# powei-lin/camera-intrinsic-calibration-rs

Measured on AMD Instinct MI355X. Metric: corner residual+Jacobian evals/sec; LM iters/sec to converge (EUCM, TUM-VI cam0), higher is better.
Workload: dtype f64

## Files before the change

### camera_intrinsic_calibration_rs_amd/csrc/ccal_api.hip

```cpp
#include <algorithm>
#include <cmath>
#include <cstdio>
#include <cstring>
#include <memory>
#include <new>

#include "ccal_internal.hpp"
#include "ccal_normal.hpp"

using namespace ccal;

#define HIP_TRY(ctx, expr)                                                                         \
    do {                                                                                           \
        hipError_t e_ = (expr);                                                                    \
        if (e_ != hipSuccess) {                                                                    \
            (ctx)->err = std::string(#expr) + ": " + hipGetErrorString(e_);                        \
            return CCAL_ERR_HIP;                                                                   \
        }                                                                                          \
    } while (0)

static void stream_synced(ccal_problem* p) {
    if (!p->nws) return;
    p->nws->tail_pending = false;
    if (p->nws->fws) p->nws->fws->tail_pending = false;
}

static int fail(ccal_ctx* ctx, int code, const char* msg) {
    if (ctx) ctx->err = msg;
    return code;
}

template <class T>
static int upload(ccal_ctx* ctx, T** dst, const T* src, size_t n) {
    HIP_TRY(ctx, hipMalloc((void**)dst, (n + 1) * sizeof(T)));
    if (n) HIP_TRY(ctx, hipMemcpyAsync(*dst, src, n * sizeof(T), hipMemcpyHostToDevice, ctx->stream));
    HIP_TRY(ctx, hipMemsetAsync(*dst + n, 0, sizeof(T), ctx->stream));
    return CCAL_OK;
}

// ... 164 lines not shown
        p->h_obs_off.assign(1, 0);
    }
    p->h_joff.resize(d->n_obs + 1);
    std::vector<uint8_t> seen((size_t)d->n_cams * (size_t)std::max(d->n_slots, 1), 0);
    int64_t j = 0;
    for (int o = 0; o < d->n_obs; ++o) {
        const int cam = p->h_obs_cam[o], slot = p->h_obs_slot[o];
        const int64_t n = p->h_obs_off[o + 1] - p->h_obs_off[o];
        if (cam < 0 || cam >= d->n_cams || slot < 0 || slot >= d->n_slots || n < 0 || p->h_obs_off[0] != 0)
            return fail(ctx, CCAL_ERR_INVALID_ARG, "bad observation frame table");
        uint8_t& sn = seen[(size_t)cam * d->n_slots + slot];
        if (sn) return fail(ctx, CCAL_ERR_INVALID_ARG, "two observation frames for the same (camera, slot)");
        sn = 1;
        p->h_joff[o] = j; j += n * 2 * p->cams[cam].D;
        p->cams[cam].obs.push_back(o);
    }
    p->h_joff[d->n_obs] = j; p->j_len = j;
    p->slot_ident = d->n_slots == d->n_obs;
    for (int o = 0; o < d->n_obs && p->slot_ident; ++o) p->slot_ident = p->h_obs_slot[o] == o;
    p->n_corners = p->h_obs_off[d->n_obs];
    if (p->n_corners >= ((int64_t)1 << 30)) return fail(ctx, CCAL_ERR_INVALID_ARG, "more than 2^30 - 1 corners in one problem: shard the frames (ccal_multi_problem_create)");
    const size_t nc = (size_t)p->n_corners;
    if (nc && (!d->p3d_x || !d->p3d_y || !d->p3d_z || !d->p2d_u || !d->p2d_v)) return fail(ctx, CCAL_ERR_INVALID_ARG, "null corner arrays");
    {
        uint32_t any = 0;
        for (size_t i = 0; i < nc; ++i) { uint32_t b; std::memcpy(&b, d->p3d_z + i, sizeof b); any |= b & 0x7fffffffu; }
        p->has_nonplanar = any != 0;
    }
    const size_t ni = (size_t)d->n_cams * CCAL_PMAX, np6 = (size_t)std::max(d->n_slots, 1) * 6, ne = (size_t)d->n_cams * 6;
    auto up256 = [](size_t b) { return (b + 255) & ~(size_t)255; };
    size_t total = 5 * up256((nc + 1) * sizeof(float)) + 2 * up256((p->h_obs_off.size() + 1) * sizeof(int64_t)) +
                   2 * up256((p->h_obs_cam.size() + 1) * sizeof(int32_t)) + 2 * (up256(ni * 8) + up256(np6 * 8) + up256(ne * 8));
    for (int c = 0; c < d->n_cams; ++c) total += up256((p->cams[c].obs.size() + 1) * sizeof(int32_t));
    std::vector<int32_t> bin_tab;
    if (d->n_cams == 1 && d->n_obs > 0) {
        std::vector<int32_t> order;
        const int m0 = p->cams[0].model;
        p->gram_bins = gram2_bin_plan(p->h_obs_off.data(), d->n_obs, m0 == kUCM || m0 == kEUCM, &order);
        if (p->gram_bins.n_bins > 0) {
            bin_tab.assign((size_t)d->n_obs * 4 + 4, 0);
            for (int i = 0; i < d->n_obs; ++i) {
                const int o = order[(size_t)i];
                bin_tab[4 * (size_t)i] = o; bin_tab[4 * (size_t)i + 1] = (int32_t)p->h_obs_off[o];
                bin_tab[4 * (size_t)i + 2] = (int32_t)(p->h_obs_off[o + 1] - p->h_obs_off[o]); bin_tab[4 * (size_t)i + 3] = p->h_obs_slot[o];
            }
            total += up256((bin_tab.size() + 1) * sizeof(int32_t));
        }
    }
    HIP_TRY(ctx, ctx_dev_alloc(ctx, (void**)&p->d_block, total));
    char* h_pack = nullptr;
    struct PackGuard { ccal_ctx* c; char*& p; ~PackGuard() { if (p) { (void)hipStreamSynchronize(c->stream); ccal::ctx_release(c, p, true); } } } pack_guard{ ctx, h_pack };
    if (total <= ((size_t)8 << 20)) HIP_TRY(ctx, ctx_host_alloc(ctx, (void**)&h_pack, total));
    if (!h_pack) HIP_TRY(ctx, hipMemsetAsync(p->d_block, 0, total, ctx->stream));
    {
        char* q = p->d_block;
        auto put = [&](auto** dst, const auto* src, size_t n) -> hipError_t {
            using T = std::remove_pointer_t<std::remove_pointer_t<decltype(dst)>>;
            *dst = reinterpret_cast<T*>(q);
            const size_t room = up256((n + 1) * sizeof(T));
            if (h_pack) {
                char* h = h_pack + (q - p->d_block);
                const size_t nb = (n && src) ? n * sizeof(T) : 0;
                if (nb) std::memcpy(h, src, nb);
                std::memset(h + nb, 0, room - nb);
                q += room;
                return hipSuccess;
            }
            q += room;
            return (n && src) ? hipMemcpyAsync(*dst, src, n * sizeof(T), hipMemcpyHostToDevice, ctx->stream) : hipSuccess;
        };
        HIP_TRY(ctx, put(&p->d_x, d->p3d_x, nc)); HIP_TRY(ctx, put(&p->d_y, d->p3d_y, nc)); HIP_TRY(ctx, put(&p->d_z, d->p3d_z, nc));
        HIP_TRY(ctx, put(&p->d_u, d->p2d_u, nc)); HIP_TRY(ctx, put(&p->d_v, d->p2d_v, nc));
        HIP_TRY(ctx, put(&p->d_obs_off, (const int64_t*)p->h_obs_off.data(), p->h_obs_off.size()));
        HIP_TRY(ctx, put(&p->d_joff, (const int64_t*)p->h_joff.data(), p->h_joff.size()));
        HIP_TRY(ctx, put(&p->d_obs_cam, (const int32_t*)p->h_obs_cam.data(), p->h_obs_cam.size()));
        HIP_TRY(ctx, put(&p->d_obs_slot, (const int32_t*)p->h_obs_slot.data(), p->h_obs_slot.size()));
        for (int c = 0; c < d->n_cams; ++c) HIP_TRY(ctx, put(&p->cams[c].d_obs, (const int32_t*)p->cams[c].obs.data(), p->cams[c].obs.size()));
        if (!bin_tab.empty()) HIP_TRY(ctx, put(&p->d_bin_tab, (const int32_t*)bin_tab.data(), bin_tab.size()));
        double** bufs[6] = { &p->d_intr, &p->d_poses, &p->d_extr, &p->d_intr_c, &p->d_poses_c, &p->d_extr_c };
        const size_t sz[6] = { ni, np6, ne, ni, np6, ne };
        const size_t packed = (size_t)(q - p->d_block);
        for (int i = 0; i < 6; ++i) { *bufs[i] = reinterpret_cast<double*>(q); q += up256(sz[i] * 8); }
        if ((size_t)(q - p->d_block) > total) return fail(ctx, CCAL_ERR_HIP, "problem block layout");
        if (h_pack) {
            HIP_TRY(ctx, hipMemcpyAsync(p->d_block, h_pack, packed, hipMemcpyHostToDevice, ctx->stream));
            HIP_TRY(ctx, hipMemsetAsync(p->d_block + packed, 0, total - packed, ctx->stream));
        }
    }
    p->lo.assign(ni, 0.0); p->hi.assign(ni, 0.0); p->has_bound.assign(ni, 0); p->fixed.assign(ni, 0);
    if (hipStreamSynchronize(ctx->stream) != hipSuccess) return fail(ctx, CCAL_ERR_HIP, "upload failed");
    p->counted = true;
    ctx->n_problems += 1;
    *out = hold.release();
    return CCAL_OK;
    CCAL_API_CATCH(ctx)
}

void ccal_problem_destroy(ccal_problem* p) {
    if (!p) return;
    if (p->nws && p->ctx && (p->nws->tail_pending || (p->nws->fws && p->nws->fws->tail_pending))) {
        (void)hipSetDevice(p->ctx->device);
        (void)hipDeviceSynchronize();
        p->nws->tail_pending = false;
        if (p->nws->fws) p->nws->fws->tail_pending = false;
    }
    ccal_ctx* ctx = p->ctx;
    if (ctx && (p->d_block || p->nws)) {
        (void)hipSetDevice(ctx->device);
        if (ctx->own_stream && ctx->stream) (void)hipStreamSynchronize(ctx->stream); else (void)hipDeviceSynchronize();
        (void)hipGetLastError();
    }
    void* ptrs[] = { p->d_block, p->d_r, p->d_J, p->d_err, p->d_scratch };
    for (void* q : ptrs) if (q) ctx_release(ctx, q, false);
    normal_ws_destroy(p);
    const bool counted = p->counted;
    delete p;
    if (ctx && counted && --ctx->n_problems == 0 && ctx->destroy_requested) ctx_free(ctx);
}

int64_t ccal_num_corners(const ccal_problem* p) { return p ? p->n_corners : -1; }
// ... 37 lines not shown
            const int at = cl.model == kOCV5 ? 4 + cv.ocv5_order[i - 4] : i;
            ccal_set_bounds(p, c, at - shift, cv.dist_lo[cl.model][i - 4], cv.dist_hi[cl.model][i - 4]);
        }
    }
    return CCAL_OK;
}
int ccal_disable_distortions(ccal_problem* p, int n_disabled, double* intr_io) {
    if (!p || n_disabled < 0) return CCAL_ERR_INVALID_ARG;
    const int shift = p->one_focal ? 1 : 0;
    for (int c = 0; c < p->n_cams; ++c) {
        for (int i = 0; i < n_disabled; ++i) {
            const int eff = p->cams[c].P - 1 - shift - i;
            if (eff < 0) return CCAL_ERR_INVALID_ARG;
            ccal_fix_param(p, c, eff);
            if (intr_io) intr_io[c * CCAL_PMAX + eff + shift] = 0.0;
        }
    }
    return CCAL_OK;
}
int ccal_set_allreduce(ccal_problem* p, ccal_allreduce_fn fn, void* user) {
    if (!p) return CCAL_ERR_INVALID_ARG;
    if (p->allreduce != fn || p->allreduce_user != user) { const int rc = drain_pending_groups(p); if (rc != CCAL_OK) return rc; }
    p->allreduce = fn; p->allreduce_user = user;
    return CCAL_OK;
}

int ccal_upload_params(ccal_problem* p, const double* intr, const double* poses, const double* extr) {
    if (!p) return CCAL_ERR_INVALID_ARG;
    ccal_ctx* ctx = p->ctx;
    HIP_TRY(ctx, hipSetDevice(ctx->device));
    if (intr) HIP_TRY(ctx, hipMemcpyAsync(p->d_intr, intr, sizeof(double) * p->n_cams * CCAL_PMAX, hipMemcpyHostToDevice, ctx->stream));
    if (poses && p->n_slots) HIP_TRY(ctx, hipMemcpyAsync(p->d_poses, poses, sizeof(double) * p->n_slots * 6, hipMemcpyHostToDevice, ctx->stream));
    if (extr) HIP_TRY(ctx, hipMemcpyAsync(p->d_extr, extr, sizeof(double) * p->n_cams * 6, hipMemcpyHostToDevice, ctx->stream));
    HIP_TRY(ctx, hipStreamSynchronize(ctx->stream));
    stream_synced(p);
    return CCAL_OK;
}
int ccal_download_params(ccal_problem* p, double* intr, double* poses, double* extr) {
    if (!p) return CCAL_ERR_INVALID_ARG;
    ccal_ctx* ctx = p->ctx;
    HIP_TRY(ctx, hipSetDevice(ctx->device));
    if (intr) HIP_TRY(ctx, hipMemcpyAsync(intr, p->d_intr, sizeof(double) * p->n_cams * CCAL_PMAX, hipMemcpyDeviceToHost, ctx->stream));
    if (poses && p->n_slots) HIP_TRY(ctx, hipMemcpyAsync(poses, p->d_poses, sizeof(double) * p->n_slots * 6, hipMemcpyDeviceToHost, ctx->stream));
    if (extr) HIP_TRY(ctx, hipMemcpyAsync(extr, p->d_extr, sizeof(double) * p->n_cams * 6, hipMemcpyDeviceToHost, ctx->stream));
    HIP_TRY(ctx, hipStreamSynchronize(ctx->stream));
    stream_synced(p);
    if (intr && p->one_focal) for (int c = 0; c < p->n_cams; ++c) intr[c * CCAL_PMAX + 1] = intr[c * CCAL_PMAX];
    return CCAL_OK;
}

static KArgs make_args(const ccal_problem* p, int cam) {
    KArgs a = {};
    a.x = p->d_x; a.y = p->d_y; a.z = p->d_z; a.u = p->d_u; a.v = p->d_v;
    a.obs_off = p->d_obs_off; a.obs_slot = p->d_obs_slot; a.joff = p->d_joff;
    a.list = p->cams[cam].d_obs; a.n_list = (int32_t)p->cams[cam].obs.size(); a.cam = cam;
    a.intr = p->d_intr; a.poses = p->d_poses; a.extr = p->d_extr;
    a.huber_delta = p->huber_delta; a.rt = model_rt(p->ctx);
    return a;
}

int ccal_eval_dev(ccal_problem* p, int apply_loss, double* r_dev, double* J_dev) {
    if (!p || !r_dev || !J_dev) return CCAL_ERR_INVALID_ARG;
    ccal_ctx* ctx = p->ctx;
    HIP_TRY(ctx, hipSetDevice(ctx->device));
    for (int c = 0; c < p->n_cams; ++c) {
        KArgs a = make_args(p, c);
        a.apply_loss = apply_loss; a.r_out = r_dev; a.J_out = J_dev;
        HIP_TRY(ctx, launch_eval(p, c, a, ctx->stream));
    }
    return CCAL_OK;
}

int ccal_eval(ccal_problem* p, const double* intr, const double* poses, const double* extr,
              int apply_loss, double* r_out, double* J_out) {
    if (!p || !intr || (!poses && p->n_slots) || (!extr && p->n_cams > 1) || !r_out || !J_out) return CCAL_ERR_INVALID_ARG;
    ccal_ctx* ctx = p->ctx;
    int rc = ccal_upload_params(p, intr, poses, extr);
    if (rc != CCAL_OK) return rc;
    if (!p->d_r) {
        HIP_TRY(ctx, ctx_dev_alloc(ctx, (void**)&p->d_r, sizeof(double) * std::max<int64_t>(2 * p->n_corners, 2)));
        HIP_TRY(ctx, test_poison_f64(ctx, p->d_r, sizeof(double) * std::max<int64_t>(2 * p->n_corners, 2), false, ctx->stream));
    }
    if (!p->d_J) {
        HIP_TRY(ctx, ctx_dev_alloc(ctx, (void**)&p->d_J, sizeof(double) * std::max<int64_t>(p->j_len, 2)));
        HIP_TRY(ctx, test_poison_f64(ctx, p->d_J, sizeof(double) * std::max<int64_t>(p->j_len, 2), false, ctx->stream));
    }
    rc = ccal_eval_dev(p, apply_loss, p->d_r, p->d_J);
    if (rc != CCAL_OK) return rc;
    if (p->n_corners) {
        HIP_TRY(ctx, hipMemcpyAsync(r_out, p->d_r, sizeof(double) * 2 * p->n_corners, hipMemcpyDeviceToHost, ctx->stream));
        HIP_TRY(ctx, hipMemcpyAsync(J_out, p->d_J, sizeof(double) * p->j_len, hipMemcpyDeviceToHost, ctx->stream));
    }
    HIP_TRY(ctx, hipStreamSynchronize(ctx->stream));
    return CCAL_OK;
}

}
// ... 76 lines not shown
```

### camera_intrinsic_calibration_rs_amd/csrc/ccal_internal.hpp

```cpp
#pragma once
#include <hip/hip_runtime.h>

#include <atomic>
#include <cstdint>
#include <exception>
#include <functional>
#include <mutex>
#include <new>
#include <string>
#include <vector>

#include "../../include/ccal.h"
#include "ccal_models.hpp"

namespace ccal {

constexpr int WAVES_PER_BLOCK = 4;
constexpr int PF_STRIDE = 64;

struct KArgs {
    const float* x; const float* y; const float* z; const float* u; const float* v;
    const int64_t* obs_off;
    const int32_t* obs_slot;
    const int64_t* joff;
    const int32_t* list;
    int32_t n_list;
    int32_t cam;
    const double* intr;
    const double* poses;
    const double* extr;
    double huber_delta;
    ModelRt rt;
    int32_t apply_loss;
    double* r_out;
    double* J_out;
    double* err_out;
};

struct NormalWs;

struct CamLayout {
    int model = 0, P = 0, Peff = 0, D = 0;
    int col_theta = 0, col_extr = -1;
    double width = 0, height = 0;
    std::vector<int32_t> obs;
    int32_t* d_obs = nullptr;
};

}

struct ccal_ctx {
    int device = 0;
    hipStream_t stream = nullptr;
    bool own_stream = false;
    std::string err;
    ccal_model_conventions conv;
    int n_problems = 0;
    bool destroy_requested = false;
    struct ccal_ctx_worker* worker = nullptr;
    char* d_batch_tab = nullptr; char* h_batch_tab = nullptr; size_t batch_tab_bytes = 0;
    std::vector<std::pair<void*, size_t>> pinned;
    struct Block { void* p; size_t bytes; };
    std::vector<Block> cache_dev, cache_host;
    std::vector<hipStream_t> cache_streams;
    std::vector<std::pair<void*, std::pair<size_t, int>>> live;
};
namespace ccal {
constexpr size_t kCacheDevMaxBytes = (size_t)1 << 30, kCacheHostMaxBytes = (size_t)64 << 20;
constexpr size_t kCacheMaxBlocks = 12;
// ... 81 lines not shown
}

namespace ccal {
constexpr int kGramMaxBins = 5;
struct GramBins {
    int32_t n_bins = 0;
    int32_t lpf[kGramMaxBins] = {}, first[kGramMaxBins] = {}, count[kGramMaxBins] = {}, wg0[kGramMaxBins + 1] = {};
    int32_t fold = 0;
};
GramBins gram2_bin_plan(const int64_t* obs_off, int n_obs, bool two_per_simd, std::vector<int32_t>* order, bool rig_list = false);

}

struct ccal_problem {
    ccal_ctx* ctx = nullptr;
    int n_cams = 0, n_slots = 0, n_obs = 0, K = 0;
    bool one_focal = false;
    double huber_delta = 1.0;
    int64_t n_corners = 0, j_len = 0;
    std::vector<ccal::CamLayout> cams;
    std::vector<int64_t> h_obs_off, h_joff;
    std::vector<int32_t> h_obs_cam, h_obs_slot;
    bool slot_ident = false;
    bool has_nonplanar = false;
    ccal::GramBins gram_bins;
    int32_t* d_bin_tab = nullptr;
    char* d_scratch = nullptr; size_t scratch_bytes = 0;
    char* d_block = nullptr;
    float *d_x = nullptr, *d_y = nullptr, *d_z = nullptr, *d_u = nullptr, *d_v = nullptr;
    int64_t *d_obs_off = nullptr, *d_joff = nullptr;
    int32_t *d_obs_cam = nullptr, *d_obs_slot = nullptr;
    double *d_intr = nullptr, *d_poses = nullptr, *d_extr = nullptr;
    double *d_intr_c = nullptr, *d_poses_c = nullptr, *d_extr_c = nullptr;
    std::vector<double> lo, hi;
    std::vector<uint8_t> has_bound, fixed;
    ccal::NormalWs* nws = nullptr;
    double *d_r = nullptr, *d_J = nullptr, *d_err = nullptr;
    ccal_allreduce_fn allreduce = nullptr;
    void* allreduce_user = nullptr;
    void* rccl_comm = nullptr;
    void* peer = nullptr;
    bool counted = false;
    bool sharded() const { return allreduce != nullptr || rccl_comm != nullptr || peer != nullptr; }
};

#define CCAL_API_TRY try {
#define CCAL_API_CATCH(ctx_expr)                                                                   \
    }                                                                                              \
    catch (const std::bad_alloc&) { ccal::note_error((ctx_expr), "out of host memory"); return CCAL_ERR_NO_MEMORY; }  \
    catch (const std::exception& e_) { ccal::note_error((ctx_expr), e_.what()); return CCAL_ERR_HIP; }                \
    catch (...) { ccal::note_error((ctx_expr), "unknown C++ exception"); return CCAL_ERR_HIP; }

namespace ccal {
inline void note_error(ccal_ctx* ctx, const char* msg) noexcept {
    if (!ctx) return;
    try { ctx->err = msg; } catch (...) { }
}
inline void note_error(const ccal_ctx*, const char*) noexcept {}
hipError_t launch_eval(const ccal_problem* p, int cam, const KArgs& a, hipStream_t s);
hipError_t launch_reproj_err(const ccal_problem* p, int cam, const KArgs& a, hipStream_t s);
int rccl_allreduce_sum(ccal_ctx* ctx, void* comm, double* buf, size_t count, hipStream_t st);
int drain_pending_groups(ccal_problem* p);
inline size_t problem_scratch_hint(const ccal_problem* p) {
    return (size_t)std::max<int64_t>(p->n_corners, 1) * 32 + (size_t)(std::max(p->n_obs, 1) + 1) * 64 + (size_t)384 * 1024;
}
hipError_t validation_stats_device(ccal_problem* p, int cam, const double* d_err, double* avg_99, double* median, hipStream_t s);
hipError_t camera_errors_device(ccal_problem* p, int cam, const double* d_err, double** d_out, int64_t* n_out, hipStream_t s);
size_t order_stats_block_bytes(int64_t n, hipStream_t s);
hipError_t order_stats_block(char* block , size_t block_bytes, int64_t n, double* avg_99, double* median, hipStream_t s);
int reprojection_errors_dev(ccal_problem* p, const double* intr, const double* poses, const double* extr);
hipError_t launch_pose_init(const ccal_problem* p, int cam, const double* d_intr, double* d_poses_obs, int32_t* d_valid,
                            int min_points, hipStream_t s);
hipError_t launch_pose_init_division(const ccal_problem* p, int cam, double lambda, double* d_poses_obs, int32_t* d_valid,
                                     int min_points, hipStream_t s);
hipError_t launch_pose_pnp(const ccal_problem* p, int cam, const double* d_intr, double* d_poses_obs, int32_t* d_valid,
                           int min_points, hipStream_t s);
hipError_t launch_pose_pnp_division(const ccal_problem* p, int cam, double lambda, double* d_poses_obs, int32_t* d_valid,
                                    int min_points, hipStream_t s);
hipError_t launch_pnp_batch(int n_prob, const int64_t* d_off, const double* d_xyz, const double* d_xn, int min_points,
                            double* d_poses, int32_t* d_n_used, double* d_cost, hipStream_t s);
struct DynLdsGuard { std::atomic<size_t> enabled[16] = {}; };
inline std::mutex& dyn_lds_mutex() { static std::mutex m; return m; }
inline hipError_t ensure_dyn_lds(const void* fn, size_t lds, DynLdsGuard& g) {
    if (lds <= 48 * 1024) return hipSuccess;
    int dev = 0;
    hipError_t e = hipGetDevice(&dev);
    if (e != hipSuccess) return e;
    std::atomic<size_t>& have = g.enabled[dev & 15];
    if (lds <= have.load(std::memory_order_acquire)) return hipSuccess;
    std::lock_guard<std::mutex> lk(dyn_lds_mutex());
    if (lds <= have.load(std::memory_order_relaxed)) return hipSuccess;
    e = hipFuncSetAttribute(fn, hipFuncAttributeMaxDynamicSharedMemorySize, (int)lds);
    if (e == hipSuccess) have.store(lds, std::memory_order_release);
// ... 25 lines not shown
```

### camera_intrinsic_calibration_rs_amd/csrc/ccal_kernels_eval.hip

```cpp
#include "ccal_device.hpp"
#include "ccal_internal.hpp"

#include <algorithm>
#include <type_traits>

namespace ccal {

__device__ __forceinline__ void wave_lds_sync() {
    __builtin_amdgcn_fence(__ATOMIC_RELEASE, "wavefront");
    __builtin_amdgcn_wave_barrier();
    __builtin_amdgcn_fence(__ATOMIC_ACQUIRE, "wavefront");
}

#ifndef CCAL_EVAL_WPB
#define CCAL_EVAL_WPB 2
#endif
#ifndef CCAL_EVAL_NT
#define CCAL_EVAL_NT 1
#endif
#ifndef CCAL_EVAL_NTR
#define CCAL_EVAL_NTR 0
#endif
#ifndef CCAL_EVAL_PREFETCH
#define CCAL_EVAL_PREFETCH -1
#endif
#ifndef CCAL_EVAL_PERSIST
#define CCAL_EVAL_PERSIST 0
#endif

constexpr int eval_tile_stride(int D) { return 2 * D + ((D & 1) ? 4 : 2); }
template <bool OTHER> constexpr int fc_doubles() { return OTHER ? FC_SIZE : FC_N0P; }

template <int MODEL, bool OF, bool OTHER, bool PF, bool AL>
__global__ __launch_bounds__(64 * CCAL_EVAL_WPB) void k_eval(const KArgs a) {
    constexpr int D = block_dim(MODEL, OF, OTHER);
    constexpr int TW = 2 * D;
    constexpr int TS = eval_tile_stride(D);
    constexpr int FCN = fc_doubles<OTHER>();
    constexpr int WS = FCN + 64 * TS;
    extern __shared__ double smem[];
    const int wave = threadIdx.x >> 6, lane = threadIdx.x & 63;
    double* fc = smem + wave * WS;
    double* tile = fc + FCN;
    const int wstride = CCAL_EVAL_PERSIST > 0 ? (int)gridDim.x * CCAL_EVAL_WPB : a.n_list;
    for (int widx = blockIdx.x * CCAL_EVAL_WPB + wave; widx < a.n_list; widx += wstride) {
    const int o = __builtin_amdgcn_readfirstlane(a.list[widx]);
    const int slot = __builtin_amdgcn_readfirstlane(a.obs_slot[o]);
    const int64_t start = a.obs_off[o];
    const int n = (int)(a.obs_off[o + 1] - start);
    const double* th_g = a.intr + a.cam * CCAL_PMAX;
    double th[th_len<MODEL>()];
    load_theta<MODEL, OF>(th_g, a.rt, th);

    float pX = 0.f, pY = 0.f, pZ = 0.f, pU = 0.f, pV = 0.f;
    if constexpr (PF) {
        if (n > 0) {
            const int64_t g0 = start + (lane < n ? lane : 0);
            pX = a.x[g0]; pY = a.y[g0]; pZ = a.z[g0]; pU = a.u[g0]; pV = a.v[g0];
        }
    }
    {
        double pose[6], ex[6];
#pragma unroll
        for (int i = 0; i < 6; ++i) pose[i] = a.poses[(int64_t)slot * 6 + i];
        if constexpr (OTHER) {
#pragma unroll
            for (int i = 0; i < 6; ++i) ex[i] = a.extr[a.cam * 6 + i];
        }
        double fcr[OTHER ? FC_SIZE : FC_N0];
        frame_setup<OTHER>(pose, ex, fcr);
        if (lane == 0) {
#pragma unroll
            for (int i = 0; i < (OTHER ? FC_SIZE : FC_N0); ++i) fc[i] = fcr[i];
        }
    }
    wave_lds_sync();

    const int64_t jbase = a.joff[o];
    auto pass = [&](auto full_tag, const int base) {
        constexpr bool FULL = decltype(full_tag)::value;
        const int c = base + lane;
        const bool valid = FULL || c < n;
        const int64_t g = start + (valid ? c : 0);
        double X, Y, Z, uo, vo;
        if constexpr (PF) {
            X = pX; Y = pY; Z = pZ; uo = pU; vo = pV;
            if (base + 64 < n) {
                const int cn = base + 64 + lane;
                const int64_t gn = start + (cn < n ? cn : 0);
                pX = a.x[gn]; pY = a.y[gn]; pZ = a.z[gn]; pU = a.u[gn]; pV = a.v[gn];
            }
        } else {
            X = a.x[g]; Y = a.y[g]; Z = a.z[g]; uo = a.u[g]; vo = a.v[g];
        }
        double ru, rv, J[TW];
        double* Ju = J;
        double* Jv = J + D;
#if defined(CCAL_EVAL_DIAG) && CCAL_EVAL_DIAG == 2
        ru = X + uo; rv = Y + vo;
#pragma unroll
        for (int i = 0; i < D; ++i) { Ju[i] = X * (double)(i + 1) + fc[0]; Jv[i] = Z * (double)(i + 1) + vo; }
#else
        corner_block<MODEL, OF, OTHER>(th, fc, X, Y, Z, uo, vo, ru, rv, Ju, Jv);
#endif
        if constexpr (AL) {
            const double sw = huber_sqrt_weight(ru * ru + rv * rv, a.huber_delta);
            ru *= sw; rv *= sw;
#pragma unroll
            for (int i = 0; i < D; ++i) { Ju[i] *= sw; Jv[i] *= sw; }
// ... 14 lines not shown
                    const int at = D0 + ocv5_pos(a.rt.ocv5_perm, i);
                    row[at] = J[D0 + i]; row[D + at] = J[D + D0 + i];
                }
            }
        }
        wave_lds_sync();
        double* dst = a.J_out + jbase + (int64_t)base * TW;
        auto put = [&](const int e) {
            const int cr = e / TW;
            const int k = e - cr * TW;
            const double2 val = *reinterpret_cast<const double2*>(tile + cr * TS + k);
#if defined(CCAL_EVAL_DIAG) && CCAL_EVAL_DIAG == 1
            if (e != lane * 2 || val.x != 12345.678) return;
#endif
#if CCAL_EVAL_NT
            __builtin_nontemporal_store(val.x, dst + e);
            __builtin_nontemporal_store(val.y, dst + e + 1);
#else
            *reinterpret_cast<double2*>(dst + e) = val;
#endif
        };
        if constexpr (FULL) {
#pragma unroll
            for (int it = 0; it < TW / 2; ++it) put(lane * 2 + 128 * it);
        } else {
            const int tot = (n - base) * TW;
            for (int e = lane * 2; e < tot; e += 128) put(e);
        }
        wave_lds_sync();
    };
    const int n_full = n & ~63;
    for (int base = 0; base < n_full; base += 64) pass(std::true_type{}, base);
    if (n_full < n) pass(std::false_type{}, n_full);
    }
}

template <int MODEL, bool OF, bool OTHER>
__global__ __launch_bounds__(256) void k_reproj_err(const KArgs a) {
    constexpr int FCN = fc_doubles<OTHER>();
    __shared__ double smem[WAVES_PER_BLOCK * FCN];
    const int wave = threadIdx.x >> 6, lane = threadIdx.x & 63;
    const int widx = blockIdx.x * WAVES_PER_BLOCK + wave;
    if (widx >= a.n_list) return;
    double* fc = smem + wave * FCN;
    const int o = __builtin_amdgcn_readfirstlane(a.list[widx]);
    const int slot = __builtin_amdgcn_readfirstlane(a.obs_slot[o]);
    const int64_t start = a.obs_off[o];
    const int n = (int)(a.obs_off[o + 1] - start);
    const double* th_g = a.intr + a.cam * CCAL_PMAX;
    double th[th_len<MODEL>()];
    load_theta<MODEL, OF>(th_g, a.rt, th);
    {
        double pose[6], ex[6];
#pragma unroll
        for (int i = 0; i < 6; ++i) pose[i] = a.poses[(int64_t)slot * 6 + i];
        if constexpr (OTHER) {
#pragma unroll
            for (int i = 0; i < 6; ++i) ex[i] = a.extr[a.cam * 6 + i];
        }
        double fcr[OTHER ? FC_SIZE : FC_N0];
        frame_setup<OTHER>(pose, ex, fcr);
        if (lane == 0) {
#pragma unroll
            for (int i = 0; i < 12; ++i) fc[i] = fcr[i];
        }
    }
    wave_lds_sync();
    for (int c = lane; c < n; c += 64) {
        const int64_t g = start + c;
        double px, py, pz, u, v;
        transform_point(fc, a.x[g], a.y[g], a.z[g], px, py, pz);
        project_uv<MODEL>(th, px, py, pz, u, v);
        const double du = u - (double)a.u[g], dv = v - (double)a.v[g];
        a.err_out[g] = sqrt(du * du + dv * dv);
    }
}

template <int MODEL, bool OF, bool OTHER, bool PF, bool AL>
static hipError_t launch_eval_pf(const KArgs& a, hipStream_t s) {
    constexpr int D = block_dim(MODEL, OF, OTHER);
    constexpr int WS = fc_doubles<OTHER>() + 64 * eval_tile_stride(D);
    const size_t lds = sizeof(double) * WS * CCAL_EVAL_WPB;
    int blocks = (a.n_list + CCAL_EVAL_WPB - 1) / CCAL_EVAL_WPB;
    if (blocks == 0) return hipSuccess;
    if (CCAL_EVAL_PERSIST > 0) blocks = std::min(blocks, 256 * CCAL_EVAL_PERSIST);
    static DynLdsGuard lds_guard;
    if (hipError_t e = ensure_dyn_lds(reinterpret_cast<const void*>(&k_eval<MODEL, OF, OTHER, PF, AL>), lds, lds_guard); e != hipSuccess) return e;
    hipLaunchKernelGGL((k_eval<MODEL, OF, OTHER, PF, AL>), dim3(blocks), dim3(64 * CCAL_EVAL_WPB), lds, s, a);
    return hipGetLastError();
}
#ifndef CCAL_EVAL_PF_MIN_D
#define CCAL_EVAL_PF_MIN_D 99
#endif
template <int MODEL, bool OF, bool OTHER> constexpr bool eval_prefetch_always() { return block_dim(MODEL, OF, OTHER) >= CCAL_EVAL_PF_MIN_D; }
template <int MODEL, bool OF, bool OTHER>
static hipError_t launch_eval_t(const KArgs& a, bool big_inputs, hipStream_t s) {
    const bool pf = CCAL_EVAL_PREFETCH < 0 ? (big_inputs || eval_prefetch_always<MODEL, OF, OTHER>()) : CCAL_EVAL_PREFETCH != 0;
    if (a.apply_loss) return pf ? launch_eval_pf<MODEL, OF, OTHER, true, true>(a, s) : launch_eval_pf<MODEL, OF, OTHER, false, true>(a, s);
    return pf ? launch_eval_pf<MODEL, OF, OTHER, true, false>(a, s) : launch_eval_pf<MODEL, OF, OTHER, false, false>(a, s);
}
template <int MODEL, bool OF, bool OTHER>
static hipError_t launch_err_t(const KArgs& a, hipStream_t s) {
    const int blocks = (a.n_list + WAVES_PER_BLOCK - 1) / WAVES_PER_BLOCK;
    if (blocks == 0) return hipSuccess;
    hipLaunchKernelGGL((k_reproj_err<MODEL, OF, OTHER>), dim3(blocks), dim3(256), 0, s, a);
    return hipGetLastError();
}

#define CCAL_DISPATCH(FN, model, of, other, ...)                                                     \
    do {                                                                                             \
        const int key_ = (model) * 4 + ((of) ? 2 : 0) + ((other) ? 1 : 0);                           \
        switch (key_) {                                                                              \
            case 0: return FN<kUCM, false, false>(__VA_ARGS__);   case 1: return FN<kUCM, false, true>(__VA_ARGS__);   \
            case 2: return FN<kUCM, true, false>(__VA_ARGS__);    case 3: return FN<kUCM, true, true>(__VA_ARGS__);    \
            case 4: return FN<kEUCM, false, false>(__VA_ARGS__);  case 5: return FN<kEUCM, false, true>(__VA_ARGS__);  \
            case 6: return FN<kEUCM, true, false>(__VA_ARGS__);   case 7: return FN<kEUCM, true, true>(__VA_ARGS__);   \
            case 8: return FN<kKB4, false, false>(__VA_ARGS__);   case 9: return FN<kKB4, false, true>(__VA_ARGS__);   \
            case 10: return FN<kKB4, true, false>(__VA_ARGS__);   case 11: return FN<kKB4, true, true>(__VA_ARGS__);   \
            case 12: return FN<kOCV5, false, false>(__VA_ARGS__); case 13: return FN<kOCV5, false, true>(__VA_ARGS__); \
            case 14: return FN<kOCV5, true, false>(__VA_ARGS__);  case 15: return FN<kOCV5, true, true>(__VA_ARGS__);  \
            default: return hipErrorInvalidValue;                                                    \
        }                                                                                            \
    } while (0)

hipError_t launch_eval(const ccal_problem* p, int cam, const KArgs& a, hipStream_t s) {
    const bool big_inputs = p->n_corners * 20 > (int64_t)120 << 20;
    CCAL_DISPATCH(launch_eval_t, p->cams[cam].model, p->one_focal, cam > 0, a, big_inputs, s);
}
hipError_t launch_reproj_err(const ccal_problem* p, int cam, const KArgs& a, hipStream_t s) {
    CCAL_DISPATCH(launch_err_t, p->cams[cam].model, p->one_focal, cam > 0, a, s);
}

}
```

### camera_intrinsic_calibration_rs_amd/csrc/ccal_solver.hip

```cpp
#include <algorithm>
#include <chrono>
#include <cmath>
#include <cstdio>
#include <cstring>

#include <cstdlib>
#include <atomic>
#include <condition_variable>
#include <functional>
#include <memory>
#include <mutex>
#include <thread>

#include "ccal_fused.hpp"
#include "ccal_devopt.hpp"

using namespace ccal;

#define HIP_TRYN(ctx, expr)                                                                        \
    do {                                                                                           \
        hipError_t e_ = (expr);                                                                    \
        if (e_ != hipSuccess) {                                                                    \
            (ctx)->err = std::string(#expr) + ": " + hipGetErrorString(e_);                        \
            return -CCAL_ERR_HIP;                                                                  \
        }                                                                                          \
    } while (0)

#define HIP_TRY(ctx, expr)                                                                         \
    do {                                                                                           \
        hipError_t e_ = (expr);                                                                    \
        if (e_ != hipSuccess) {                                                                    \
            (ctx)->err = std::string(#expr) + ": " + hipGetErrorString(e_);                        \
            return CCAL_ERR_HIP;                                                                   \
        }                                                                                          \
    } while (0)

namespace ccal {

hipError_t test_poison_f64(ccal_ctx* ctx, void* p, size_t bytes, bool host, hipStream_t s) {
#ifdef CCAL_TEST_HOOKS
    const char* e = std::getenv("CCAL_TEST_POISON_ALLOC");
    if (!e || e[0] != '1' || !p || !bytes) return hipSuccess;
    if (host) { std::memset(p, 0xFF, bytes); return hipSuccess; }
    return hipMemsetAsync(p, 0xFF, bytes, s ? s : ctx->stream);
#else
    (void)ctx; (void)p; (void)bytes; (void)host; (void)s;
    return hipSuccess;
#endif
}

void normal_ws_destroy(ccal_problem* p) {
    NormalWs* w = p->nws;
    if (!w) return;
    if (w->tail_pending || (w->fws && w->fws->tail_pending)) {
        (void)hipSetDevice(p->ctx->device);
        (void)hipDeviceSynchronize();
    }
    void* ptrs[] = { w->G[0], w->G[1], w->cost_o[0], w->cost_o[1], w->d_goff, w->d_slot_off, w->d_slot_obs, w->d_obs_cam,
                     w->d_caminfo, w->partial, w->red, w->pf, w->dc, w->mc_slot, w->scal, w->flags, w->cols, w->d_slot_desc, w->d_slot_rec, w->d_all_obs, w->d_obs_owner };
    ccal_ctx* ctx = p->ctx;
    for (void* q : ptrs) if (q) ctx_release(ctx, q, false);
    for (int32_t* q : w->d_gen_sorted) if (q) ctx_release(ctx, q, false);
    if (w->h_pinned) (void)hipHostFree(w->h_pinned);
    if (w->d_gstate) ctx_release(ctx, w->d_gstate, false);
    if (w->side) { (void)hipStreamSynchronize(w->side); ctx_stream_put(ctx, w->side); }
    if (w->h_gstatus) ctx_release(ctx, w->h_gstatus, true);
    if (w->h_gstate) (void)hipHostFree(w->h_gstate);
    if (FusedWs* f = w->fws) {
        if (f->side) { (void)hipStreamSynchronize(f->side); ctx_stream_put(ctx, f->side); }
        if (f->d_block) ctx_release(ctx, f->d_block, false);
        if (f->h_block) ctx_release(ctx, f->h_block, true);
        if (f->fcbuf) (void)hipFree(f->fcbuf);
        delete f;
    }
    delete w;
    p->nws = nullptr;
}

int drain_pending_groups(ccal_problem* p) {
    NormalWs* w = p->nws;
    if (!w || !(w->tail_pending || (w->fws && w->fws->tail_pending))) return CCAL_OK;
    ccal_ctx* ctx = p->ctx;
// ... 391 lines not shown
    const bool lm = o->method == CCAL_METHOD_LM;
    s->radius = o->lm_initial_radius; s->dec = 2.0;
    s->lambda = lm ? 1.0 / o->lm_initial_radius : 0.0;
    s->lambda_spec = lm ? 1.0 / lm_radius_cap(o->lm_initial_radius) : 0.0;
    s->min_error = o->min_error; s->min_abs = o->min_abs_error_decrease; s->min_rel = o->min_rel_error_decrease;
    s->cur = 0; s->first = 1; s->max_iter = o->max_iterations; s->method = o->method;
    s->error_metric = o->error_metric ? 1 : 0;
}
static int max_groups_for(const ccal_solver_opts* o) {
    const int64_t n = (int64_t)(o->method == CCAL_METHOD_LM ? 2 : 1) * std::max(o->max_iterations, 0) + 2;
    return (int)std::min<int64_t>(n, kMaxGroups);
}
static int groups_in_flight(const ccal_problem* p, const char* env_name) {
    if (p->allreduce && !p->rccl_comm && !p->peer) {
        static const int hook_depth = std::max(1, dev_env_int("CCAL_FUSED_DEPTH_HOOK", 1));
        return hook_depth;
    }
    return std::max(1, dev_env_int(env_name, 2));
}

struct SolveJob {
    ccal_problem* p; const ccal_solver_opts* o; bool host_io;
    double* intr_io; double* poses_io; double* extr_io;
    ccal_ctx* ctx; NormalWs* w; hipStream_t st;
    std::chrono::steady_clock::time_point t0, t_wait;
    std::vector<int> pending;
    int enq = 0, max_groups = 0, depth = 1, seq = 0;
    long spins = 0;
    bool finished = false, enqueued_any = false;
    double timeout_s = 30.0;
    const std::atomic<int>* cancel = nullptr;
    int share = 1;
    SolveJob(ccal_problem* p_, const ccal_solver_opts* o_, bool hio, double* i, double* po, double* e)
        : p(p_), o(o_), host_io(hio), intr_io(i), poses_io(po), extr_io(e), ctx(p_->ctx), w(p_->nws), st(p_->ctx->stream) {}
    virtual ~SolveJob() {}
    virtual int begin() = 0;
    virtual int enqueue() = 0;
    virtual HostStatus* status() = 0;
    virtual const DevState* dev_state() = 0;
    virtual void mark_tail_pending() = 0;
    virtual int end(ccal_report* rep) = 0;
    int fail_enqueued(int code) { mark_tail_pending(); return code; }
    int fill() {
        while ((int)pending.size() < depth && enq < max_groups) {
            const int sq = enqueue();
            if (sq < 0) return enqueued_any ? fail_enqueued(-sq) : -sq;
            enqueued_any = true;
            if (pending.empty()) t_wait = std::chrono::steady_clock::now();
            pending.push_back(sq); ++enq;
        }
        return CCAL_OK;
    }
    int poll(bool* fin) {
        *fin = finished;
        if (finished) return CCAL_OK;
        if (cancel && cancel->load(std::memory_order_acquire)) { ctx->err = "sharded solve: a peer shard failed"; return fail_enqueued(CCAL_ERR_HIP); }
        int rc = fill();
        if (rc != CCAL_OK) return rc;
        if (pending.empty()) { finished = true; *fin = true; return CCAL_OK; }
        const int waited = pending.front();
        bool arrived = false;
        HostStatus* hst = status();
        if ((rc = check_status(ctx, st, hst, dev_state(), waited, timeout_s, t_wait, &spins, &arrived)) != CCAL_OK) return fail_enqueued(rc);
        if (!arrived) return CCAL_OK;
        pending.erase(pending.begin());
        t_wait = std::chrono::steady_clock::now(); spins = 0;
        const uint64_t wd = hst->word;
// ... 139 lines not shown
            }
            HIP_TRYN(ctx, launch_gram_iter(p->cams[0].model, p->one_focal, fa, st));
            if (fa.n_part != iter_rows) { ctx->err = "single-launch group: row count changed"; return -CCAL_ERR_INVALID_ARG; }
            return sq;
        }
        if (sharded) {
            if (p->peer) {
                fa.red = f->red + (size_t)inproc_parity(p->peer) * f->red_stride;
                HIP_TRYN(ctx, enqueue_fused_system(p, fa, schur_m, st));
                if (inproc_post(p->peer, fa.red, (size_t)f->RB1, (void*)st, &ha.peers) != 0) { ctx->err = "in-process transport: a peer shard failed or did not arrive"; return -CCAL_ERR_HIP; }
            } else {
                HIP_TRYN(ctx, enqueue_fused_system(p, fa, schur_m, st));
                if (int e = allreduce(p, f->red, (size_t)f->RB1); e != CCAL_OK) return -e;
            }
            ha.partial = nullptr; ha.n_part = 0;
        } else {
            HIP_TRYN(ctx, enqueue_fused_gram_schur(p, fa, schur_m, st));
            if (fa.n_part <= head_reduce_max_rows) { ha.partial = f->partial; ha.n_part = fa.n_part; }
            else { HIP_TRYN(ctx, launch_reduce1(fa, st)); ha.partial = nullptr; ha.n_part = 0; }
        }
        ha.seq = ++seq;
        HIP_TRYN(ctx, launch_head(ha, st));
        return seq;
    }
    int end(ccal_report* rep) override {
        HostStatus* hst = f->h_status;
        hipStream_t dl = st;
        if (status_done(hst->word) && (!pending.empty() || zero_copy || !host_io)) { dl = f->side; f->tail_pending = true; }
        else HIP_TRY(ctx, hipStreamSynchronize(st));
        struct { int done, iter, cur, acc, rej, hits, misses; double cur_cost, initial_cost; } ds =
            { status_done(hst->word), hst->iter, hst->cur, hst->lm_accepted, hst->lm_rejected, hst->spec_hits, hst->spec_misses, hst->cur_cost, hst->initial_cost };
        const int status = ds.done ? ds.done - 1 : CCAL_ERR_NO_CONVERGENCE;
        if (ds.cur == 1) { std::swap(p->d_intr, p->d_intr_c); std::swap(p->d_poses, p->d_poses_c); }
        ccal_report R = {};
        R.status = status; R.iterations = ds.iter; R.lm_accepted = ds.acc; R.lm_rejected = ds.rej;
        R.lm_spec_hits = ds.hits; R.lm_spec_misses = ds.misses;
        R.initial_cost = ds.initial_cost; R.final_cost = ds.cur_cost;
        if (host_io) {
            if (zero_copy && ds.done) {
                std::memcpy(intr_io, const_cast<const double*>(f->h_result), CCAL_PMAX * sizeof(double));
                if (!(spread && pinned_dev)) std::memcpy(poses_io, const_cast<const double*>(f->h_result) + CCAL_PMAX, np6 * sizeof(double));
            } else if (pinned_dev) {
                double* h_intr = h_poses;
                HIP_TRY(ctx, hipMemcpyAsync(poses_io, p->d_poses, np6 * sizeof(double), hipMemcpyDeviceToHost, dl));
                HIP_TRY(ctx, hipMemcpyAsync(h_intr, p->d_intr, CCAL_PMAX * sizeof(double), hipMemcpyDeviceToHost, dl));
                HIP_TRY(ctx, hipStreamSynchronize(dl));
                std::memcpy(intr_io, h_intr, CCAL_PMAX * sizeof(double));
            } else {
                double* h_intr = h_poses + np6;
                if (np6) HIP_TRY(ctx, hipMemcpyAsync(h_poses, p->d_poses, np6 * sizeof(double), hipMemcpyDeviceToHost, dl));
                HIP_TRY(ctx, hipMemcpyAsync(h_intr, p->d_intr, CCAL_PMAX * sizeof(double), hipMemcpyDeviceToHost, dl));
                HIP_TRY(ctx, hipStreamSynchronize(dl));
                std::memcpy(poses_io, h_poses, np6 * sizeof(double));
                std::memcpy(intr_io, h_intr, CCAL_PMAX * sizeof(double));
            }
            if (p->one_focal) intr_io[1] = intr_io[0];
        }
        R.solve_ms = std::chrono::duration<double, std::milli>(std::chrono::steady_clock::now() - t0).count();
        if (rep) *rep = R;
        if (status == CCAL_ERR_NOT_PD) ctx->err = "normal equations are not positive definite";
        return status;
    }
};

struct GeneralJob : SolveJob {
    using SolveJob::SolveJob;
// ... 25 lines not shown
        timeout_s = wait_timeout(p, o);
        return fill();
    }
    int enqueue() override {
        const double min_d = o->lm_min_diagonal, max_d = o->lm_max_diagonal;
        DevState* ds = w->d_gstate;
        HIP_TRYN(ctx, launch_gram_dev_all(p, ds, st));
        HIP_TRYN(ctx, launch_schur(p, w->cur, 0.0, min_d, max_d, st, ds));
        if (p->peer) {
            w->red_out = w->red + (size_t)inproc_parity(p->peer) * (size_t)(w->RB + 8);
            HIP_TRYN(ctx, launch_reduce(p, st, ds));
            const int bad = inproc_post(p->peer, w->red_out, (size_t)w->RB, (void*)st, &w->peers);
            w->red_out = nullptr;
            if (bad) { w->peers.n = 0; ctx->err = "in-process transport: a peer shard failed or did not arrive"; return -CCAL_ERR_HIP; }
        } else {
            HIP_TRYN(ctx, launch_reduce(p, st, ds));
            if (int e = allreduce(p, w->red, (size_t)w->RB); e != CCAL_OK) return -e;
        }
        HIP_TRYN(ctx, launch_solve(p, 0.0, min_d, max_d, st, ds, w->h_gstatus, ++seq, o->verbose != 0));
        w->peers.n = 0;
        if (!w->gen_backsub) HIP_TRYN(ctx, launch_backsub(p, 0.0, min_d, max_d, st, ds));
        return seq;
    }
    int end(ccal_report* rep) override {
        HostStatus* hst = w->h_gstatus;
        hipStream_t dl = st;
        if (status_done(hst->word) && !pending.empty()) { dl = w->side; w->tail_pending = true; }
        else HIP_TRY(ctx, hipStreamSynchronize(st));
        const int status = status_done(hst->word) ? status_done(hst->word) - 1 : CCAL_ERR_NO_CONVERGENCE;
        if (hst->cur == 1) {
            std::swap(p->d_intr, p->d_intr_c); std::swap(p->d_poses, p->d_poses_c); std::swap(p->d_extr, p->d_extr_c);
            w->cur ^= 1;
        }
        ccal_report R = {};
        R.status = status; R.iterations = hst->iter; R.lm_accepted = hst->lm_accepted; R.lm_rejected = hst->lm_rejected;
        R.lm_spec_hits = hst->spec_hits; R.lm_spec_misses = hst->spec_misses;
        R.initial_cost = hst->initial_cost; R.final_cost = hst->cur_cost;
        if (host_io) {
            HIP_TRY(ctx, hipMemcpyAsync(intr_io, p->d_intr, sizeof(double) * p->n_cams * CCAL_PMAX, hipMemcpyDeviceToHost, dl));
            if (poses_io && p->n_slots) HIP_TRY(ctx, hipMemcpyAsync(poses_io, p->d_poses, sizeof(double) * p->n_slots * 6, hipMemcpyDeviceToHost, dl));
            if (extr_io) HIP_TRY(ctx, hipMemcpyAsync(extr_io, p->d_extr, sizeof(double) * p->n_cams * 6, hipMemcpyDeviceToHost, dl));
            HIP_TRY(ctx, hipStreamSynchronize(dl));
            if (p->one_focal) for (int c = 0; c < p->n_cams; ++c) intr_io[c * CCAL_PMAX + 1] = intr_io[c * CCAL_PMAX];
        }
        R.solve_ms = std::chrono::duration<double, std::milli>(std::chrono::steady_clock::now() - t0).count();
        if (rep) *rep = R;
        if (status == CCAL_ERR_NOT_PD) ctx->err = "normal equations are not positive definite";
        return status;
    }
};

static bool use_fused_path(const ccal_problem* p) { return p->n_cams == 1 && !dev_env("CCAL_DISABLE_FUSED"); }

extern "C" {

#ifdef CCAL_STAMPS
int ccal_debug_fcbuf(ccal_problem* p, double* out, int64_t n) {
    if (!p || !p->nws || !out) return CCAL_ERR_INVALID_ARG;
    if (!p->nws->fws) {
        const NormalWs* w = p->nws;
        if (!w->general_ready) return CCAL_OK;
        const int64_t room = (int64_t)w->RB * (std::max(w->n_pw, w->n_rows) - w->n_rows), m = std::min(n, room);
        if (m > 0 && hipMemcpy(out, w->partial + (int64_t)w->RB * w->n_rows, m * sizeof(double), hipMemcpyDeviceToHost) != hipSuccess) return CCAL_ERR_HIP;
        return CCAL_OK;
    }
    const int64_t m = std::min<int64_t>(n, (int64_t)std::max(p->n_obs, 1) * 40);
    if (hipMemcpy(out, p->nws->fws->fcbuf, m * sizeof(double), hipMemcpyDeviceToHost) != hipSuccess) return CCAL_ERR_HIP;
    return CCAL_OK;
}
#endif

int ccal_build_normal_dev(ccal_problem* p, double lambda) {
    if (!p) return CCAL_ERR_INVALID_ARG;
    CCAL_API_TRY
    HIP_TRY(p->ctx, hipSetDevice(p->ctx->device));
    int rc = normal_ws_ensure(p);
    if (rc != CCAL_OK) return rc;
    NormalWs* w = p->nws;
    w->red_fused = false;
    if (p->n_cams == 1 && p->n_obs > 0 && !p->sharded() && !dev_env("CCAL_DISABLE_FUSED")) {
        ccal_ctx* ctx = p->ctx;
        if ((rc = fused_ws_ensure(p)) != CCAL_OK) return rc;
        FusedWs* f = w->fws;
        hipStream_t st = ctx->stream;
        if (f->tail_pending) { HIP_TRY(ctx, hipStreamSynchronize(st)); f->tail_pending = false; }
        FusedArgs fa = make_fused_args(p, 1e-6, 1e32);
        const bool schur_m = fused_use_schur1m(p, fa);
        if (!(f->state_is_eval && f->state_eval_lambda == lambda)) {
            HIP_TRY(ctx, launch_state_eval(f->d_state, lambda, st));
            f->state_is_eval = true; f->state_eval_lambda = lambda;
        }
        HIP_TRY(ctx, enqueue_fused_system(p, fa, schur_m, st));
        w->red_fused = true;
        return CCAL_OK;
    }
    if ((rc = normal_ws_ensure_general(p)) != CCAL_OK) return rc;
    if (w->tail_pending) { HIP_TRY(p->ctx, hipStreamSynchronize(p->ctx->stream)); w->tail_pending = false; }
    if ((rc = enqueue_gram(p, false, w->cur)) != CCAL_OK) return rc;
    return enqueue_reduce_system(p, w->cur, lambda, 1e-6, 1e32);
    CCAL_API_CATCH(p->ctx)
}

// ... 452 lines not shown
```

Baseline: 27.66 billion.

## Precompute per-frame pose constants in a separate kernel and cache across evals

Adds a k_frame_consts kernel that computes per-observation frame setup (rotation and derived constants) into a device table once per pose version. The eval kernel then loads these constants into registers through scalar/constant loads instead of recomputing frame_setup in every wave and syncing through LDS. A version counter skips the precompute when poses have not changed between eval calls. This removes redundant per-wave transcendental work and an LDS sync, and lowers LDS use. The cost is an extra small launch plus table memory, and it relies on the version tracking staying correct.

Measured after the change: 27.27 billion. 1.4% lower.

```diff
diff --git a/camera_intrinsic_calibration_rs_amd/csrc/ccal_api.hip b/camera_intrinsic_calibration_rs_amd/csrc/ccal_api.hip
--- a/camera_intrinsic_calibration_rs_amd/csrc/ccal_api.hip
+++ b/camera_intrinsic_calibration_rs_amd/csrc/ccal_api.hip
@@ -5,6 +5,7 @@
 #include <memory>
 #include <new>
 
+#include "ccal_device.hpp"
 #include "ccal_internal.hpp"
 #include "ccal_normal.hpp"
 
@@ -235,6 +236,9 @@
     size_t total = 5 * up256((nc + 1) * sizeof(float)) + 2 * up256((p->h_obs_off.size() + 1) * sizeof(int64_t)) +
                    2 * up256((p->h_obs_cam.size() + 1) * sizeof(int32_t)) + 2 * (up256(ni * 8) + up256(np6 * 8) + up256(ne * 8));
     for (int c = 0; c < d->n_cams; ++c) total += up256((p->cams[c].obs.size() + 1) * sizeof(int32_t));
+    p->fc_stride = d->n_cams > 1 ? FC_SIZE : FC_N0P;
+    const size_t nfc = (size_t)std::max(d->n_obs, 1) * (size_t)p->fc_stride;
+    total += up256(nfc * 8);
     std::vector<int32_t> bin_tab;
     if (d->n_cams == 1 && d->n_obs > 0) {
         std::vector<int32_t> order;
@@ -284,11 +288,13 @@
         const size_t sz[6] = { ni, np6, ne, ni, np6, ne };
         const size_t packed = (size_t)(q - p->d_block);
         for (int i = 0; i < 6; ++i) { *bufs[i] = reinterpret_cast<double*>(q); q += up256(sz[i] * 8); }
+        p->d_fc = reinterpret_cast<double*>(q); q += up256(nfc * 8);
         if ((size_t)(q - p->d_block) > total) return fail(ctx, CCAL_ERR_HIP, "problem block layout");
         if (h_pack) {
             HIP_TRY(ctx, hipMemcpyAsync(p->d_block, h_pack, packed, hipMemcpyHostToDevice, ctx->stream));
             HIP_TRY(ctx, hipMemsetAsync(p->d_block + packed, 0, total - packed, ctx->stream));
         }
+        HIP_TRY(ctx, test_poison_f64(ctx, p->d_fc, nfc * 8, false, ctx->stream));
     }
     p->lo.assign(ni, 0.0); p->hi.assign(ni, 0.0); p->has_bound.assign(ni, 0); p->fixed.assign(ni, 0);
     if (hipStreamSynchronize(ctx->stream) != hipSuccess) return fail(ctx, CCAL_ERR_HIP, "upload failed");
@@ -392,6 +398,7 @@
     if (intr) HIP_TRY(ctx, hipMemcpyAsync(p->d_intr, intr, sizeof(double) * p->n_cams * CCAL_PMAX, hipMemcpyHostToDevice, ctx->stream));
     if (poses && p->n_slots) HIP_TRY(ctx, hipMemcpyAsync(p->d_poses, poses, sizeof(double) * p->n_slots * 6, hipMemcpyHostToDevice, ctx->stream));
     if (extr) HIP_TRY(ctx, hipMemcpyAsync(p->d_extr, extr, sizeof(double) * p->n_cams * 6, hipMemcpyHostToDevice, ctx->stream));
+    if ((poses && p->n_slots) || extr) p->params_written();
     HIP_TRY(ctx, hipStreamSynchronize(ctx->stream));
     stream_synced(p);
     return CCAL_OK;
@@ -416,6 +423,7 @@
     a.list = p->cams[cam].d_obs; a.n_list = (int32_t)p->cams[cam].obs.size(); a.cam = cam;
     a.intr = p->d_intr; a.poses = p->d_poses; a.extr = p->d_extr;
     a.huber_delta = p->huber_delta; a.rt = model_rt(p->ctx);
+    a.fc = p->d_fc; a.fc_stride = p->fc_stride;
     return a;
 }
 
@@ -423,6 +431,12 @@
     if (!p || !r_dev || !J_dev) return CCAL_ERR_INVALID_ARG;
     ccal_ctx* ctx = p->ctx;
     HIP_TRY(ctx, hipSetDevice(ctx->device));
+    hipStreamCaptureStatus cap = hipStreamCaptureStatusNone;
+    HIP_TRY(ctx, hipStreamIsCapturing(ctx->stream, &cap));
+    if (cap != hipStreamCaptureStatusNone || p->fc_version != p->pose_version) {
+        HIP_TRY(ctx, launch_frame_consts(p, ctx->stream));
+        p->fc_version = cap != hipStreamCaptureStatusNone ? 0 : p->pose_version;
+    }
     for (int c = 0; c < p->n_cams; ++c) {
         KArgs a = make_args(p, c);
         a.apply_loss = apply_loss; a.r_out = r_dev; a.J_out = J_dev;
diff --git a/camera_intrinsic_calibration_rs_amd/csrc/ccal_internal.hpp b/camera_intrinsic_calibration_rs_amd/csrc/ccal_internal.hpp
--- a/camera_intrinsic_calibration_rs_amd/csrc/ccal_internal.hpp
+++ b/camera_intrinsic_calibration_rs_amd/csrc/ccal_internal.hpp
@@ -35,6 +35,8 @@
     double* r_out;
     double* J_out;
     double* err_out;
+    const double* fc;
+    int32_t fc_stride;
 };
 
 struct NormalWs;
@@ -182,6 +184,10 @@
     int32_t *d_obs_cam = nullptr, *d_obs_slot = nullptr;
     double *d_intr = nullptr, *d_poses = nullptr, *d_extr = nullptr;
     double *d_intr_c = nullptr, *d_poses_c = nullptr, *d_extr_c = nullptr;
+    double* d_fc = nullptr;
+    int fc_stride = 0;
+    uint64_t pose_version = 1, fc_version = 0;
+    void params_written() { ++pose_version; }
     std::vector<double> lo, hi;
     std::vector<uint8_t> has_bound, fixed;
     ccal::NormalWs* nws = nullptr;
@@ -207,8 +213,10 @@
     try { ctx->err = msg; } catch (...) { }
 }
 inline void note_error(const ccal_ctx*, const char*) noexcept {}
-hipError_t launch_eval(const ccal_problem* p, int cam, const KArgs& a, hipStream_t s);
+__attribute__((visibility("hidden"))) hipError_t launch_eval(const ccal_problem* p, int cam, const KArgs& a, hipStream_t s);
 hipError_t launch_reproj_err(const ccal_problem* p, int cam, const KArgs& a, hipStream_t s);
+__attribute__((visibility("hidden"))) hipError_t launch_frame_consts(const ccal_problem* p, hipStream_t s);
+__attribute__((visibility("hidden"))) void test_count_fc_launch();
 int rccl_allreduce_sum(ccal_ctx* ctx, void* comm, double* buf, size_t count, hipStream_t st);
 int drain_pending_groups(ccal_problem* p);
 inline size_t problem_scratch_hint(const ccal_problem* p) {
diff --git a/camera_intrinsic_calibration_rs_amd/csrc/ccal_kernels_eval.hip b/camera_intrinsic_calibration_rs_amd/csrc/ccal_kernels_eval.hip
--- a/camera_intrinsic_calibration_rs_amd/csrc/ccal_kernels_eval.hip
+++ b/camera_intrinsic_calibration_rs_amd/csrc/ccal_kernels_eval.hip
@@ -30,22 +30,55 @@
 
 constexpr int eval_tile_stride(int D) { return 2 * D + ((D & 1) ? 4 : 2); }
 template <bool OTHER> constexpr int fc_doubles() { return OTHER ? FC_SIZE : FC_N0P; }
-
-template <int MODEL, bool OF, bool OTHER, bool PF, bool AL>
+#ifdef CCAL_LEGACY_KERNELS
+constexpr bool kEvalChain = true;
+#else
+constexpr bool kEvalChain = false;
+#endif
+template <bool OTHER> constexpr int eval_lds_fc() { return kEvalChain ? fc_doubles<OTHER>() : 0; }
+
+__global__ __launch_bounds__(256) void k_frame_consts(const int32_t* __restrict__ obs_slot, const int32_t* __restrict__ obs_cam,
+                                                      const double* __restrict__ poses, const double* __restrict__ extr,
+                                                      double* __restrict__ fc_tab, int fc_stride, int n_obs) {
+    const int o = blockIdx.x * 256 + threadIdx.x;
+    if (o >= n_obs) return;
+    const int cam = obs_cam[o];
+    const int64_t slot = obs_slot[o];
+    double pose[6], ex[6];
+#pragma unroll
+    for (int i = 0; i < 6; ++i) pose[i] = poses[slot * 6 + i];
+    double* dst = fc_tab + (int64_t)o * fc_stride;
+    if (cam == 0) {
+        double fcr[FC_N0P];
+        frame_setup<false>(pose, nullptr, fcr);
+        fcr[FC_N0] = 0.0;
+#pragma unroll
+        for (int i = 0; i < FC_N0P; i += 2) *reinterpret_cast<double2*>(dst + i) = make_double2(fcr[i], fcr[i + 1]);
+    } else {
+#pragma unroll
+        for (int i = 0; i < 6; ++i) ex[i] = extr[cam * 6 + i];
+        double fcr[FC_SIZE];
+        frame_setup<true>(pose, ex, fcr);
+#pragma unroll
+        for (int i = 0; i < FC_SIZE; i += 2) *reinterpret_cast<double2*>(dst + i) = make_double2(fcr[i], fcr[i + 1]);
+    }
+}
+
+template <int MODEL, bool OF, bool OTHER, bool PF, bool AL, bool CHAIN = kEvalChain>
 __global__ __launch_bounds__(64 * CCAL_EVAL_WPB) void k_eval(const KArgs a) {
     constexpr int D = block_dim(MODEL, OF, OTHER);
     constexpr int TW = 2 * D;
     constexpr int TS = eval_tile_stride(D);
     constexpr int FCN = fc_doubles<OTHER>();
-    constexpr int WS = FCN + 64 * TS;
+    constexpr int WS = eval_lds_fc<OTHER>() + 64 * TS;
     extern __shared__ double smem[];
     const int wave = threadIdx.x >> 6, lane = threadIdx.x & 63;
-    double* fc = smem + wave * WS;
-    double* tile = fc + FCN;
+    double* tile = smem + wave * WS + eval_lds_fc<OTHER>();
     const int wstride = CCAL_EVAL_PERSIST > 0 ? (int)gridDim.x * CCAL_EVAL_WPB : a.n_list;
-    for (int widx = blockIdx.x * CCAL_EVAL_WPB + wave; widx < a.n_list; widx += wstride) {
+    int widx = blockIdx.x * CCAL_EVAL_WPB + wave;
+    if (widx >= a.n_list) return;
+    do {
     const int o = __builtin_amdgcn_readfirstlane(a.list[widx]);
-    const int slot = __builtin_amdgcn_readfirstlane(a.obs_slot[o]);
     const int64_t start = a.obs_off[o];
     const int n = (int)(a.obs_off[o + 1] - start);
     const double* th_g = a.intr + a.cam * CCAL_PMAX;
@@ -59,7 +92,11 @@
             pX = a.x[g0]; pY = a.y[g0]; pZ = a.z[g0]; pU = a.u[g0]; pV = a.v[g0];
         }
     }
-    {
+    double fcs[CHAIN ? 1 : FCN];
+    const double* fc = fcs;
+    if constexpr (CHAIN) {
+        const int slot = __builtin_amdgcn_readfirstlane(a.obs_slot[o]);
+        double* fcl = smem + wave * WS;
         double pose[6], ex[6];
 #pragma unroll
         for (int i = 0; i < 6; ++i) pose[i] = a.poses[(int64_t)slot * 6 + i];
@@ -71,10 +108,16 @@
         frame_setup<OTHER>(pose, ex, fcr);
         if (lane == 0) {
 #pragma unroll
-            for (int i = 0; i < (OTHER ? FC_SIZE : FC_N0); ++i) fc[i] = fcr[i];
-        }
-    }
-    wave_lds_sync();
+            for (int i = 0; i < (OTHER ? FC_SIZE : FC_N0); ++i) fcl[i] = fcr[i];
+        }
+        fc = fcl;
+        wave_lds_sync();
+    } else {
+        typedef const double __attribute__((address_space(4))) cdouble;
+        cdouble* src = (cdouble*)(a.fc + (int64_t)o * a.fc_stride);
+#pragma unroll
+        for (int i = 0; i < FCN; ++i) fcs[i] = src[i];
+    }
 
     const int64_t jbase = a.joff[o];
     auto pass = [&](auto full_tag, const int base) {
@@ -155,7 +198,8 @@
     const int n_full = n & ~63;
     for (int base = 0; base < n_full; base += 64) pass(std::true_type{}, base);
     if (n_full < n) pass(std::false_type{}, n_full);
-    }
+    widx += wstride;
+    } while (CCAL_EVAL_PERSIST > 0 && widx < a.n_list);
 }
 
 template <int MODEL, bool OF, bool OTHER>
@@ -202,7 +246,7 @@
 template <int MODEL, bool OF, bool OTHER, bool PF, bool AL>
 static hipError_t launch_eval_pf(const KArgs& a, hipStream_t s) {
     constexpr int D = block_dim(MODEL, OF, OTHER);
-    constexpr int WS = fc_doubles<OTHER>() + 64 * eval_tile_stride(D);
+    constexpr int WS = eval_lds_fc<OTHER>() + 64 * eval_tile_stride(D);
     const size_t lds = sizeof(double) * WS * CCAL_EVAL_WPB;
     int blocks = (a.n_list + CCAL_EVAL_WPB - 1) / CCAL_EVAL_WPB;
     if (blocks == 0) return hipSuccess;
@@ -250,6 +294,13 @@
     const bool big_inputs = p->n_corners * 20 > (int64_t)120 << 20;
     CCAL_DISPATCH(launch_eval_t, p->cams[cam].model, p->one_focal, cam > 0, a, big_inputs, s);
 }
+hipError_t launch_frame_consts(const ccal_problem* p, hipStream_t s) {
+    if (p->n_obs == 0) return hipSuccess;
+    test_count_fc_launch();
+    hipLaunchKernelGGL(k_frame_consts, dim3((p->n_obs + 255) / 256), dim3(256), 0, s, p->d_obs_slot, p->d_obs_cam, p->d_poses, p->d_extr,
+                       p->d_fc, p->fc_stride, p->n_obs);
+    return hipGetLastError();
+}
 hipError_t launch_reproj_err(const ccal_problem* p, int cam, const KArgs& a, hipStream_t s) {
     CCAL_DISPATCH(launch_err_t, p->cams[cam].model, p->one_focal, cam > 0, a, s);
 }
diff --git a/camera_intrinsic_calibration_rs_amd/csrc/ccal_solver.hip b/camera_intrinsic_calibration_rs_amd/csrc/ccal_solver.hip
--- a/camera_intrinsic_calibration_rs_amd/csrc/ccal_solver.hip
+++ b/camera_intrinsic_calibration_rs_amd/csrc/ccal_solver.hip
@@ -48,6 +48,13 @@
     return hipSuccess;
 #endif
 }
+
+#ifdef CCAL_TEST_HOOKS
+static std::atomic<int64_t> g_fc_launches{0};
+void test_count_fc_launch() { g_fc_launches.fetch_add(1, std::memory_order_relaxed); }
+#else
+void test_count_fc_launch() {}
+#endif
 
 void normal_ws_destroy(ccal_problem* p) {
     NormalWs* w = p->nws;
@@ -505,7 +512,9 @@
     const std::atomic<int>* cancel = nullptr;
     int share = 1;
     SolveJob(ccal_problem* p_, const ccal_solver_opts* o_, bool hio, double* i, double* po, double* e)
-        : p(p_), o(o_), host_io(hio), intr_io(i), poses_io(po), extr_io(e), ctx(p_->ctx), w(p_->nws), st(p_->ctx->stream) {}
+        : p(p_), o(o_), host_io(hio), intr_io(i), poses_io(po), extr_io(e), ctx(p_->ctx), w(p_->nws), st(p_->ctx->stream) {
+        p->params_written();
+    }
     virtual ~SolveJob() {}
     virtual int begin() = 0;
     virtual int enqueue() = 0;
@@ -711,6 +720,7 @@
             { status_done(hst->word), hst->iter, hst->cur, hst->lm_accepted, hst->lm_rejected, hst->spec_hits, hst->spec_misses, hst->cur_cost, hst->initial_cost };
         const int status = ds.done ? ds.done - 1 : CCAL_ERR_NO_CONVERGENCE;
         if (ds.cur == 1) { std::swap(p->d_intr, p->d_intr_c); std::swap(p->d_poses, p->d_poses_c); }
+        p->params_written();
         ccal_report R = {};
         R.status = status; R.iterations = ds.iter; R.lm_accepted = ds.acc; R.lm_rejected = ds.rej;
         R.lm_spec_hits = ds.hits; R.lm_spec_misses = ds.misses;
@@ -802,6 +812,7 @@
             std::swap(p->d_intr, p->d_intr_c); std::swap(p->d_poses, p->d_poses_c); std::swap(p->d_extr, p->d_extr_c);
             w->cur ^= 1;
         }
+        p->params_written();
         ccal_report R = {};
         R.status = status; R.iterations = hst->iter; R.lm_accepted = hst->lm_accepted; R.lm_rejected = hst->lm_rejected;
         R.lm_spec_hits = hst->spec_hits; R.lm_spec_misses = hst->spec_misses;
@@ -838,6 +849,10 @@
     if (hipMemcpy(out, p->nws->fws->fcbuf, m * sizeof(double), hipMemcpyDeviceToHost) != hipSuccess) return CCAL_ERR_HIP;
     return CCAL_OK;
 }
+#endif
+
+#ifdef CCAL_TEST_HOOKS
+int64_t ccal_test_fc_launches(void) { return ccal::g_fc_launches.load(std::memory_order_relaxed); }
 #endif
 
 int ccal_build_normal_dev(ccal_problem* p, double lambda) {
```
